# NikolaZubic/2dimageto3dmodel

Hardware: NVIDIA H100
Metric: render+loss+GAN images/sec (cfg3: cfg2 render+loss at batch 32 + conv-GAN 256x256 G/D iteration, 1 G : 2 D, Adam) (higher is better)
Workload: dtype tf32 (convs) / f32

## Files before the change

2dimageto3dmodel_b200/csrc/b3d_core.cu:

```cuda
#include <atomic>
#include <stdarg.h>
#include <string.h>

#include "b3d_common.cuh"

namespace b3d {
static thread_local char g_err[512] = "";
static thread_local char g_variant[256] = "";
static std::atomic<uint64_t> g_launches{0};

void set_error(const char* fmt, ...) {
    va_list ap;
    va_start(ap, fmt);
    vsnprintf(g_err, sizeof(g_err), fmt, ap);
    va_end(ap);
}
void clear_variant() { g_variant[0] = 0; }
void add_variant(const char* fmt, ...) {
    size_t n = strlen(g_variant);
    if (n + 2 >= sizeof(g_variant)) return;
    if (n) g_variant[n++] = ';';
    va_list ap;
    va_start(ap, fmt);
    vsnprintf(g_variant + n, sizeof(g_variant) - n, fmt, ap);
    va_end(ap);
}
void count_launch(int n) { g_launches.fetch_add((uint64_t)n, std::memory_order_relaxed); }
}

extern "C" {
const char* b3d_last_error(void) { return b3d::g_err; }
const char* b3d_last_variant(void) { return b3d::g_variant; }
int b3d_version(void) { return 420; }
uint64_t b3d_launch_count(void) { return b3d::g_launches.load(std::memory_order_relaxed); }
}
```

2dimageto3dmodel_b200/csrc/tc_common.cuh:

```cuda
#pragma once
#include <cuda.h>
#include <cuda_runtime.h>
#include <stdint.h>

#include "b3d_common.cuh"

namespace tc {

__device__ __forceinline__ uint32_t smem_u32(const void* p) { return (uint32_t)__cvta_generic_to_shared(p); }

__device__ __forceinline__ void mbar_init(uint64_t* bar, uint32_t count) {
    asm volatile("mbarrier.init.shared::cta.b64 [%0], %1;" ::"r"(smem_u32(bar)), "r"(count));
}
__device__ __forceinline__ void fence_barrier_init() { asm volatile("fence.mbarrier_init.release.cluster;" ::: "memory"); }
__device__ __forceinline__ void fence_proxy_async() { asm volatile("fence.proxy.async.shared::cta;" ::: "memory"); }

__device__ __forceinline__ void mbar_arrive_expect_tx(uint64_t* bar, uint32_t bytes) {
    asm volatile("mbarrier.arrive.expect_tx.shared::cta.b64 _, [%0], %1;" ::"r"(smem_u32(bar)), "r"(bytes) : "memory");
}
__device__ __forceinline__ void mbar_arrive(uint64_t* bar) {
    asm volatile("mbarrier.arrive.shared::cta.b64 _, [%0];" ::"r"(smem_u32(bar)) : "memory");
}
__device__ __forceinline__ void mbar_arrive(uint64_t* bar, uint32_t count) {
    asm volatile("mbarrier.arrive.shared::cta.b64 _, [%0], %1;" ::"r"(smem_u32(bar)), "r"(count) : "memory");
// ... 52 lines not shown
    return v;
}
__device__ __forceinline__ float lds_f32(uint32_t smem_addr) {
    float v;
    asm volatile("ld.shared.f32 %0, [%1];" : "=f"(v) : "r"(smem_addr) : "memory");
    return v;
}
__device__ __forceinline__ float2 lds_f32x2(uint32_t smem_addr) {
    float2 v;
    asm volatile("ld.shared.v2.f32 {%0, %1}, [%2];" : "=f"(v.x), "=f"(v.y) : "r"(smem_addr) : "memory");
    return v;
}
__device__ __forceinline__ float4 lds_f32x4(uint32_t smem_addr) {
    float4 v;
    asm volatile("ld.shared.v4.f32 {%0, %1, %2, %3}, [%4];" : "=f"(v.x), "=f"(v.y), "=f"(v.z), "=f"(v.w) : "r"(smem_addr) : "memory");
    return v;
}
__device__ __forceinline__ void sts_f32x4(uint32_t smem_addr, float a, float b, float c, float d) {
    asm volatile("st.shared.v4.f32 [%0], {%1, %2, %3, %4};" ::"r"(smem_addr), "f"(a), "f"(b), "f"(c), "f"(d) : "memory");
}
__device__ __forceinline__ void fence_operand(uint32_t& r) { asm volatile("" : "+r"(r)::"memory"); }
__device__ __forceinline__ void fence_operand(float& r) { asm volatile("" : "+f"(r)::"memory"); }
template <int N>
__device__ __forceinline__ void setmaxnreg_dec() { asm volatile("setmaxnreg.dec.sync.aligned.u32 %0;" ::"n"(N)); }
template <int N>
__device__ __forceinline__ void setmaxnreg_inc() { asm volatile("setmaxnreg.inc.sync.aligned.u32 %0;" ::"n"(N)); }

template <int N>
struct Wgmma;
template <>
struct Wgmma<64> {
    __device__ __forceinline__ static void mma_rs(float (&d)[32], const uint32_t (&a)[4], uint64_t db, uint32_t accumulate) {
        asm volatile(
            "{\n"
            ".reg .pred p;\n"
            "setp.ne.b32 p, %37, 0;\n"
            "wgmma.mma_async.sync.aligned.m64n64k8.f32.tf32.tf32 "
            "{%0, %1, %2, %3, %4, %5, %6, %7, %8, %9, %10, %11, %12, %13, %14, %15, %16, %17, %18, %19, %20, %21, %22, %23, %24, %25, %26, %27, %28, %29, %30, %31}, "
            "{%32, %33, %34, %35}, %36, p, 1, 1;\n"
            "}\n"
            : "+f"(d[0]), "+f"(d[1]), "+f"(d[2]), "+f"(d[3]), "+f"(d[4]), "+f"(d[5]), "+f"(d[6]), "+f"(d[7]), "+f"(d[8]), "+f"(d[9]), "+f"(d[10]), "+f"(d[11]), "+f"(d[12]), "+f"(d[13]), "+f"(d[14]), "+f"(d[15]), "+f"(d[16]), "+f"(d[17]), "+f"(d[18]), "+f"(d[19]), "+f"(d[20]), "+f"(d[21]), "+f"(d[22]), "+f"(d[23]), "+f"(d[24]), "+f"(d[25]), "+f"(d[26]), "+f"(d[27]), "+f"(d[28]), "+f"(d[29]), "+f"(d[30]), "+f"(d[31])
            : "r"(a[0]), "r"(a[1]), "r"(a[2]), "r"(a[3]), "l"(db), "r"(accumulate));
    }
    __device__ __forceinline__ static void mma(float (&d)[32], uint64_t da, uint64_t db, uint32_t accumulate) {
        asm volatile(
            "{\n"
            ".reg .pred p;\n"
            "setp.ne.b32 p, %34, 0;\n"
            "wgmma.mma_async.sync.aligned.m64n64k8.f32.tf32.tf32 "
            "{%0, %1, %2, %3, %4, %5, %6, %7, %8, %9, %10, %11, %12, %13, %14, %15, %16, %17, %18, %19, %20, %21, %22, %23, %24, %25, %26, %27, %28, %29, %30, %31}, "
            "%32, %33, p, 1, 1;\n"
            "}\n"
            : "+f"(d[0]), "+f"(d[1]), "+f"(d[2]), "+f"(d[3]), "+f"(d[4]), "+f"(d[5]), "+f"(d[6]), "+f"(d[7]), "+f"(d[8]), "+f"(d[9]), "+f"(d[10]), "+f"(d[11]), "+f"(d[12]), "+f"(d[13]), "+f"(d[14]), "+f"(d[15]), "+f"(d[16]), "+f"(d[17]), "+f"(d[18]), "+f"(d[19]), "+f"(d[20]), "+f"(d[21]), "+f"(d[22]), "+f"(d[23]), "+f"(d[24]), "+f"(d[25]), "+f"(d[26]), "+f"(d[27]), "+f"(d[28]), "+f"(d[29]), "+f"(d[30]), "+f"(d[31])
            : "l"(da), "l"(db), "r"(accumulate));
    }
};
template <>
struct Wgmma<128> {
    __device__ __forceinline__ static void mma_rs(float (&d)[64], const uint32_t (&a)[4], uint64_t db, uint32_t accumulate) {
        asm volatile(
            "{\n"
            ".reg .pred p;\n"
            "setp.ne.b32 p, %69, 0;\n"
            "wgmma.mma_async.sync.aligned.m64n128k8.f32.tf32.tf32 "
            "{%0, %1, %2, %3, %4, %5, %6, %7, %8, %9, %10, %11, %12, %13, %14, %15, %16, %17, %18, %19, %20, %21, %22, %23, %24, %25, %26, %27, %28, %29, %30, %31, %32, %33, %34, %35, %36, %37, %38, %39, %40, %41, %42, %43, %44, %45, %46, %47, %48, %49, %50, %51, %52, %53, %54, %55, %56, %57, %58, %59, %60, %61, %62, %63}, "
            "{%64, %65, %66, %67}, %68, p, 1, 1;\n"
            "}\n"
            : "+f"(d[0]), "+f"(d[1]), "+f"(d[2]), "+f"(d[3]), "+f"(d[4]), "+f"(d[5]), "+f"(d[6]), "+f"(d[7]), "+f"(d[8]), "+f"(d[9]), "+f"(d[10]), "+f"(d[11]), "+f"(d[12]), "+f"(d[13]), "+f"(d[14]), "+f"(d[15]), "+f"(d[16]), "+f"(d[17]), "+f"(d[18]), "+f"(d[19]), "+f"(d[20]), "+f"(d[21]), "+f"(d[22]), "+f"(d[23]), "+f"(d[24]), "+f"(d[25]), "+f"(d[26]), "+f"(d[27]), "+f"(d[28]), "+f"(d[29]), "+f"(d[30]), "+f"(d[31]), "+f"(d[32]), "+f"(d[33]), "+f"(d[34]), "+f"(d[35]), "+f"(d[36]), "+f"(d[37]), "+f"(d[38]), "+f"(d[39]), "+f"(d[40]), "+f"(d[41]), "+f"(d[42]), "+f"(d[43]), "+f"(d[44]), "+f"(d[45]), "+f"(d[46]), "+f"(d[47]), "+f"(d[48]), "+f"(d[49]), "+f"(d[50]), "+f"(d[51]), "+f"(d[52]), "+f"(d[53]), "+f"(d[54]), "+f"(d[55]), "+f"(d[56]), "+f"(d[57]), "+f"(d[58]), "+f"(d[59]), "+f"(d[60]), "+f"(d[61]), "+f"(d[62]), "+f"(d[63])
            : "r"(a[0]), "r"(a[1]), "r"(a[2]), "r"(a[3]), "l"(db), "r"(accumulate));
    }
    __device__ __forceinline__ static void mma(float (&d)[64], uint64_t da, uint64_t db, uint32_t accumulate) {
        asm volatile(
            "{\n"
            ".reg .pred p;\n"
            "setp.ne.b32 p, %66, 0;\n"
            "wgmma.mma_async.sync.aligned.m64n128k8.f32.tf32.tf32 "
            "{%0, %1, %2, %3, %4, %5, %6, %7, %8, %9, %10, %11, %12, %13, %14, %15, %16, %17, %18, %19, %20, %21, %22, %23, %24, %25, %26, %27, %28, %29, %30, %31, %32, %33, %34, %35, %36, %37, %38, %39, %40, %41, %42, %43, %44, %45, %46, %47, %48, %49, %50, %51, %52, %53, %54, %55, %56, %57, %58, %59, %60, %61, %62, %63}, "
            "%64, %65, p, 1, 1;\n"
            "}\n"
            : "+f"(d[0]), "+f"(d[1]), "+f"(d[2]), "+f"(d[3]), "+f"(d[4]), "+f"(d[5]), "+f"(d[6]), "+f"(d[7]), "+f"(d[8]), "+f"(d[9]), "+f"(d[10]), "+f"(d[11]), "+f"(d[12]), "+f"(d[13]), "+f"(d[14]), "+f"(d[15]), "+f"(d[16]), "+f"(d[17]), "+f"(d[18]), "+f"(d[19]), "+f"(d[20]), "+f"(d[21]), "+f"(d[22]), "+f"(d[23]), "+f"(d[24]), "+f"(d[25]), "+f"(d[26]), "+f"(d[27]), "+f"(d[28]), "+f"(d[29]), "+f"(d[30]), "+f"(d[31]), "+f"(d[32]), "+f"(d[33]), "+f"(d[34]), "+f"(d[35]), "+f"(d[36]), "+f"(d[37]), "+f"(d[38]), "+f"(d[39]), "+f"(d[40]), "+f"(d[41]), "+f"(d[42]), "+f"(d[43]), "+f"(d[44]), "+f"(d[45]), "+f"(d[46]), "+f"(d[47]), "+f"(d[48]), "+f"(d[49]), "+f"(d[50]), "+f"(d[51]), "+f"(d[52]), "+f"(d[53]), "+f"(d[54]), "+f"(d[55]), "+f"(d[56]), "+f"(d[57]), "+f"(d[58]), "+f"(d[59]), "+f"(d[60]), "+f"(d[61]), "+f"(d[62]), "+f"(d[63])
            : "l"(da), "l"(db), "r"(accumulate));
    }
};
__device__ __forceinline__ uint64_t desc_k128(uint32_t smem_addr) {
    uint64_t d = 0;
    d |= (uint64_t)((smem_addr & 0x3FFFF) >> 4);
    d |= (uint64_t)1 << 16;
    d |= (uint64_t)(1024 >> 4) << 32;
    d |= (uint64_t)1 << 62;
    return d;
}
__device__ __forceinline__ uint64_t desc_k32(uint32_t smem_addr) {
    uint64_t d = 0;
    d |= (uint64_t)((smem_addr & 0x3FFFF) >> 4);
    d |= (uint64_t)1 << 16;
    d |= (uint64_t)(256 >> 4) << 32;
    d |= (uint64_t)3 << 62;
    return d;
}

typedef CUresult (*EncodeTiledFn)(CUtensorMap*, CUtensorMapDataType, cuuint32_t, void*, const cuuint64_t*,
                                  const cuuint64_t*, const cuuint32_t*, const cuuint32_t*, CUtensorMapInterleave,
                                  CUtensorMapSwizzle, CUtensorMapL2promotion, CUtensorMapFloatOOBfill);

inline EncodeTiledFn encode_fn() {
    static EncodeTiledFn fn = nullptr;
    if (!fn) {
        void* p = nullptr;
        cudaDriverEntryPointQueryResult q;
        if (cudaGetDriverEntryPoint("cuTensorMapEncodeTiled", &p, cudaEnableDefault, &q) == cudaSuccess &&
            q == cudaDriverEntryPointSuccess)
            fn = reinterpret_cast<EncodeTiledFn>(p);
    }
    return fn;
}

inline int make_tmap_f32(CUtensorMap* m, const void* base, int rank, const uint64_t* dims, const uint64_t* strides_b,
                         const uint32_t* box, const uint32_t* elem_strides = nullptr,
                         CUtensorMapSwizzle swz = CU_TENSOR_MAP_SWIZZLE_128B) {
    EncodeTiledFn fn = encode_fn();
    if (!fn) {
        b3d::set_error("cuTensorMapEncodeTiled is not available from the driver");
        return B3D_ECUDA;
    }
    cuuint64_t gd[5], gs[5];
    cuuint32_t bx[5], es[5];
    for (int i = 0; i < rank; ++i) {
        gd[i] = dims[i];
        bx[i] = box[i];
        es[i] = elem_strides ? elem_strides[i] : 1;
        if (i > 0) gs[i - 1] = strides_b[i - 1];
    }
    CUresult r = fn(m, CU_TENSOR_MAP_DATA_TYPE_FLOAT32, (cuuint32_t)rank, const_cast<void*>(base), gd, gs, bx, es,
                    CU_TENSOR_MAP_INTERLEAVE_NONE, swz, CU_TENSOR_MAP_L2_PROMOTION_L2_256B,
                    CU_TENSOR_MAP_FLOAT_OOB_FILL_NONE);
    if (r != CUDA_SUCCESS) {
        b3d::set_error("cuTensorMapEncodeTiled failed with CUresult %d (rank %d, inner box %u)", (int)r, rank, box[0]);
        return B3D_ECUDA;
    }
    return B3D_OK;
}

inline int num_sms() {
    int dev = 0, n = 0;
    if (cudaGetDevice(&dev) != cudaSuccess || cudaDeviceGetAttribute(&n, cudaDevAttrMultiProcessorCount, dev) != cudaSuccess || n < 1)
        return 132;
    return n;
}

}
```

2dimageto3dmodel_b200/csrc/tc_conv.cu:

```cuda
#include "tc_common.cuh"

namespace {

constexpr int BM = 128;
constexpr int BK = 32;
constexpr int MMA_K = 8;
constexpr int MAX_TAPS = 25;
constexpr int NTHREADS = 384;

struct ConvParams {
    int N, Hout, Wout, Cout;
    int BW, BH, BI;
    int tiles_x, tiles_y;
    int xbase;
    int ntaps, kslices;
    int sy, sx;
    int dy[MAX_TAPS], dx[MAX_TAPS];
    int wtap[MAX_TAPS];
    int OH, OW, OC, osy, osx;
    float leaky;
    double* stats;
    int fold;
    int fold_y0;
    int mask;
// ... 420 lines not shown
    const int wg = threadIdx.x >> 7, tid = threadIdx.x & 127;

    if (wg == 0) {
        tc::setmaxnreg_dec<80>();
        auto issue = [&](int j) {
            if (tid != 0) return;
            const long long k = k_lo + j;
            const int n = (int)(k / per_img), rem = (int)(k % per_img);
            const int x0 = (rem % p.kx) * p.BWk, y0 = (rem / p.kx) * p.BHk;
            const int rb = j % NRAW;
            unsigned char* dst = raw + rb * S::RAW_BYTES;
            tc::mbar_wait(rawempty + rb, ((j / NRAW) & 1) ^ 1);
            tc::mbar_arrive_expect_tx(rawfull + rb, S::DY_BYTES + S::RAW_X);
            tc::tma_load_5d(dst, &tmap_dy, rawfull + rb, 0, x0, y0, n, co0 / 32);
            tc::tma_load_5d(dst + S::DY_BYTES, &tmap_x, rawfull + rb, 0, p.st * x0 + s + p.xoff, p.st * y0 + r - p.pad_y, n, ci0 / 32);
        };
        for (int j = 0; j < NRAW - 1 && j < KI; ++j) issue(j);
        const uint32_t raw_s = tc::smem_u32(raw), base_s = tc::smem_u32(base);
        for (int it = 0; it < KI; ++it) {
            if (it + NRAW - 1 < KI) issue(it + NRAW - 1);
            const int rb = it % NRAW, st = it % STAGES;
            tc::mbar_wait(rawfull + rb, (it / NRAW) & 1);
            tc::mbar_wait(empty + st, ((it / STAGES) & 1) ^ 1);
            wgrad_transpose<BN, T, S::WROWS>(raw_s + rb * S::RAW_BYTES + S::DY_BYTES, base_s + st * S::STAGE_BYTES, tid);
            tc::fence_proxy_async();
            tc::mbar_arrive(full + st);
            tc::named_sync(2, 128);
        }
        return;
    }
    tc::setmaxnreg_inc<208>();

    const int h = wg - 1, lane = tid & 31;
    if (h >= nact) return;
    int aoff[4];
#pragma unroll
    for (int e = 0; e < 4; ++e)
        aoff[e] = dy_tile_offset(h * 64 + wgrad_row_co((tid >> 5) * 16 + (lane >> 2) + 8 * (e & 1)), (lane & 3) + 4 * (e >> 1));
    float acc[T][BN / 2];
#pragma unroll
    for (int t = 0; t < T; ++t)
#pragma unroll
        for (int i = 0; i < BN / 2; ++i) acc[t][i] = 0.f;
    wgrad_consume<BN, T, STAGES, NRAW, S::RAW_BYTES, S::STAGE_BYTES>(acc, tc::smem_u32(raw), tc::smem_u32(base), full, empty, rawfull,
                                                                     rawempty, aoff, 0, 1, KI, tid, true);
    if (KI == 0) return;
    const int m_a = (tid >> 5) * 16 + (lane >> 2);
    const int cq = ci0 + 2 * (lane & 3);
#pragma unroll
    for (int t = 0; t < T; ++t) {
        const int sc = s + t * p.tstep;
#pragma unroll
        for (int e = 0; e < 2; ++e) {
            const int co = co0 + h * 64 + wgrad_row_co(m_a + 8 * e);
            if (co >= p.Cout) continue;
#pragma unroll
            for (int j = 0; j < BN / 8; ++j) {
                const int ci = cq + 8 * j;
                if (ci >= p.Cin) continue;
                const float v0 = acc[t][4 * j + 2 * e], v1 = acc[t][4 * j + 2 * e + 1];
                if (p.tapmajor) {
                    atomicAdd(reinterpret_cast<float2*>(dw + ((size_t)(r * p.kw + sc) * p.Cout + co) * p.Cin + ci), make_float2(v0, v1));
                } else {
                    atomicAdd(dw + (((size_t)co * p.Cin + ci) * p.kh + r) * p.kw + sc, v0);
                    atomicAdd(dw + (((size_t)co * p.Cin + ci + 1) * p.kh + r) * p.kw + sc, v1);
                }
            }
        }
    }
}

template <int BN, int STAGES, int NRAW, int T>
int launch_wgrad(const CUtensorMap& mdy, const CUtensorMap& mx, const WgradParams& p, float* dw, dim3 grid, cudaStream_t st) {
    using S = WSmem<BN, STAGES, NRAW, T>;
    static_assert(S::TOTAL <= 227 * 1024, "wgrad pipeline does not fit shared memory");
    B3D_CUDA_OK(cudaFuncSetAttribute(wgrad_wgmma_kernel<BN, STAGES, NRAW, T>, cudaFuncAttributeMaxDynamicSharedMemorySize, S::TOTAL));
    wgrad_wgmma_kernel<BN, STAGES, NRAW, T><<<grid, NTHREADS, S::TOTAL, st>>>(mdy, mx, p, dw);
    B3D_LAUNCH_OK();
    b3d::add_variant("wgrad_wgmma<%d,%d,%d,%d>", BN, STAGES, NRAW, T);
    return B3D_OK;
}

constexpr int STEM_KW = 5, STEM_STAGES = 4, STEM_NRAW = 3;
constexpr int STEM_BATCH = 3;
struct StemSmem {
    static constexpr int DY_BYTES = 64 * BK * 4;
    static constexpr int WPX = BK + STEM_KW - 1;
    static constexpr int RAW_X_MAX = 8 * WPX * 32;
    static constexpr int RAW_BYTES = (DY_BYTES + RAW_X_MAX + 1023) / 1024 * 1024;
    static constexpr int TILE_BYTES = 64 * BK * 4;
    static constexpr int STAGE_BYTES = STEM_KW * TILE_BYTES;
    static constexpr int TOTAL = STEM_STAGES * STAGE_BYTES + STEM_NRAW * RAW_BYTES + 1024 + 256;
};

__global__ void __launch_bounds__(NTHREADS, 1)
wgrad_stem_kernel(const __grid_constant__ CUtensorMap tmap_dy, const __grid_constant__ CUtensorMap tmap_x,
                  const WgradParams p, int fold_kh, float* __restrict__ dw) {
    using S = StemSmem;
    extern __shared__ unsigned char smem_raw[];
    unsigned char* base = reinterpret_cast<unsigned char*>((reinterpret_cast<uintptr_t>(smem_raw) + 1023) & ~uintptr_t(1023));
    unsigned char* raw = base + STEM_STAGES * S::STAGE_BYTES;
    uint64_t* full = reinterpret_cast<uint64_t*>(raw + STEM_NRAW * S::RAW_BYTES);
    uint64_t* empty = full + STEM_STAGES;
    uint64_t* rawfull = empty + STEM_STAGES;
    uint64_t* rawempty = rawfull + STEM_NRAW;

    const int co0 = blockIdx.x * 64, split = blockIdx.y;
    const int per_img = p.kx * p.ky;
    const long long ktotal = (long long)p.N * per_img;
    const long long k_lo = ktotal * split / p.splits, k_hi = ktotal * (split + 1) / p.splits;
    const int KI = (int)(k_hi - k_lo);
    const int creal = 8 * fold_kh;
    const int xbytes = fold_kh * S::WPX * 32;

    if (threadIdx.x == 0) {
        tc::tma_prefetch_desc(&tmap_dy);
        tc::tma_prefetch_desc(&tmap_x);
        for (int i = 0; i < STEM_STAGES; ++i) {
            tc::mbar_init(full + i, 128);
            tc::mbar_init(empty + i, 1);
        }
        for (int i = 0; i < STEM_NRAW; ++i) {
            tc::mbar_init(rawfull + i, 1);
            tc::mbar_init(rawempty + i, 4);
        }
        tc::fence_barrier_init();
    }
    __syncthreads();
    const int wg = threadIdx.x >> 7, tid = threadIdx.x & 127;

    if (wg == 0) {
        tc::setmaxnreg_dec<56>();
        auto issue = [&](int j) {
            if (tid != 0) return;
            const long long k = k_lo + j;
            const int n = (int)(k / per_img), rem = (int)(k % per_img);
            const int x0 = (rem % p.kx) * BK, y0 = rem / p.kx;
            const int rb = j % STEM_NRAW;
            unsigned char* dst = raw + rb * S::RAW_BYTES;
            tc::mbar_wait(rawempty + rb, ((j / STEM_NRAW) & 1) ^ 1);
            tc::mbar_arrive_expect_tx(rawfull + rb, S::DY_BYTES + xbytes);
            tc::tma_load_5d(dst, &tmap_dy, rawfull + rb, 0, x0, y0, n, co0 / 32);
            tc::tma_load_4d(dst + S::DY_BYTES, &tmap_x, rawfull + rb, 0, x0, y0 - p.pad_y, n);
        };
        for (int i = tid; i < STEM_STAGES * STEM_KW * (64 - creal) * 8; i += 128) {
            const int c = creal + (i >> 3) % (64 - creal), tile = (i >> 3) / (64 - creal);
            *reinterpret_cast<float4*>(base + tile * S::TILE_BYTES + c * 128 + (i & 7) * 16) = make_float4(0.f, 0.f, 0.f, 0.f);
        }
        for (int j = 0; j < STEM_NRAW - 1 && j < KI; ++j) issue(j);
        const int ntask = fold_kh * 8 * STEM_KW * 8;
        const uint32_t raw_s = tc::smem_u32(raw), base_s = tc::smem_u32(base);
        for (int it = 0; it < KI; ++it) {
            if (it + STEM_NRAW - 1 < KI) issue(it + STEM_NRAW - 1);
            const int rb = it % STEM_NRAW, st = it % STEM_STAGES;
            tc::mbar_wait(rawfull + rb, (it / STEM_NRAW) & 1);
            tc::mbar_wait(empty + st, ((it / STEM_STAGES) & 1) ^ 1);
            const uint32_t src = raw_s + rb * S::RAW_BYTES + S::DY_BYTES;
            const uint32_t dst = base_s + st * S::STAGE_BYTES;
            for (int i0 = tid; i0 < ntask; i0 += STEM_BATCH * 128) {
                float v[STEM_BATCH][4];
                uint32_t d[STEM_BATCH];
#pragma unroll
                for (int g = 0; g < STEM_BATCH; ++g) {
                    const int i = i0 + 128 * g;
                    if (i >= ntask) break;
                    const int ci = i & 7, u = i >> 3;
                    const int s = u % STEM_KW, q = (u / STEM_KW) & 7, r = u / (STEM_KW * 8);
                    const uint32_t a = src + ((r * S::WPX + 4 * q + s) * 8 + ci) * 4;
#pragma unroll
                    for (int e = 0; e < 4; ++e) v[g][e] = tc::lds_f32(a + 32 * e);
                    d[g] = dst + s * S::TILE_BYTES + (8 * r + ci) * 128 + ((q ^ ci) << 4);
                }
#pragma unroll
                for (int g = 0; g < STEM_BATCH; ++g) {
                    if (i0 + 128 * g >= ntask) break;
                    tc::sts_f32x4(d[g], v[g][0], v[g][1], v[g][2], v[g][3]);
                }
            }
            tc::fence_proxy_async();
            tc::mbar_arrive(full + st);
            tc::named_sync(2, 128);
        }
        return;
    }
    tc::setmaxnreg_inc<224>();

    const int h = wg - 1, lane = tid & 31;
    int aoff[4];
#pragma unroll
    for (int e = 0; e < 4; ++e)
        aoff[e] = dy_tile_offset(wgrad_row_co((tid >> 5) * 16 + (lane >> 2) + 8 * (e & 1)), (lane & 3) + 4 * (e >> 1));
    float acc[STEM_KW][32];
#pragma unroll
    for (int t = 0; t < STEM_KW; ++t)
#pragma unroll
        for (int i = 0; i < 32; ++i) acc[t][i] = 0.f;
    static_assert(S::TILE_BYTES == 64 * 128, "a tap's B tile is 64 channel rows of 128 bytes");
    wgrad_consume<64, STEM_KW, STEM_STAGES, STEM_NRAW, S::RAW_BYTES, S::STAGE_BYTES>(acc, tc::smem_u32(raw), tc::smem_u32(base), full, empty,
                                                                                     rawfull, rawempty, aoff, h, 2, KI, tid, false);
    if (h >= KI) return;
    const int m_a = (tid >> 5) * 16 + (lane >> 2);
#pragma unroll
    for (int t = 0; t < STEM_KW; ++t) {
#pragma unroll
        for (int e = 0; e < 2; ++e) {
            const int co = co0 + wgrad_row_co(m_a + 8 * e);
#pragma unroll
            for (int j = 0; j < 8; ++j) {
                const int ci = 8 * j + 2 * (lane & 3);
                if (ci >= creal) continue;
                const float v0 = acc[t][4 * j + 2 * e], v1 = acc[t][4 * j + 2 * e + 1];
                if (p.tapmajor) {
                    atomicAdd(reinterpret_cast<float2*>(dw + ((size_t)t * p.Cout + co) * p.Cin + ci), make_float2(v0, v1));
                } else {
                    atomicAdd(dw + ((size_t)co * p.Cin + ci) * STEM_KW + t, v0);
                    atomicAdd(dw + ((size_t)co * p.Cin + ci + 1) * STEM_KW + t, v1);
                }
            }
        }
    }
}

int wgrad_splits(int base_ctas, long long ktotal) {
    constexpr long long FIXED = 16;
    const long long sms = tc::num_sms();
    long long smax = ktotal / 8;
    if (smax > 8 * sms) smax = 8 * sms;
    int best = 1;
    long long best_cost = -1;
    for (long long s = 1; s <= smax; ++s) {
        const long long cost = (base_ctas * s + sms - 1) / sms * ((ktotal + s - 1) / s + FIXED);
        if (best_cost < 0 || cost < best_cost) { best = (int)s; best_cost = cost; }
    }
    return best;
}

template <int BN, int STAGES, int KW = 1>
int launch_conv(const CUtensorMap& mx, const CUtensorMap& mw, const CUtensorMap& mm, const ConvParams& p, const float* bias, float* out,
                int tiles, cudaStream_t st) {
    using S = CSmem<BN, STAGES, KW>;
    static_assert(S::TOTAL <= 227 * 1024, "conv pipeline does not fit shared memory");
    B3D_CUDA_OK(cudaFuncSetAttribute(conv_wgmma_kernel<BN, STAGES, KW>, cudaFuncAttributeMaxDynamicSharedMemorySize, S::TOTAL));
    const int work = tiles * b3d::ceil_div(p.Cout, BN) * p.ncls;
    const int sms = tc::num_sms();
    conv_wgmma_kernel<BN, STAGES, KW><<<work < sms ? work : sms, NTHREADS, S::TOTAL, st>>>(mx, mw, mm, p, bias, out, tiles, work);
    B3D_LAUNCH_OK();
    if (KW > 1) b3d::add_variant("conv_wgmma_rowwin<%d,%d,%d>", BN, KW, STAGES);
    else b3d::add_variant("conv_wgmma<%d,%d>", BN, STAGES);
    return B3D_OK;
}

template <int BN>
int launch_rowwin(int kw, const CUtensorMap& mx, const CUtensorMap& mw, const CUtensorMap& mm, const ConvParams& p, const float* bias,
                  float* out, int tiles, cudaStream_t st) {
    if (kw == 2) return launch_conv<BN, BN == 64 ? 5 : 4, 2>(mx, mw, mm, p, bias, out, tiles, st);
    if (kw == 3) return launch_conv<BN, BN == 64 ? 4 : 3, 3>(mx, mw, mm, p, bias, out, tiles, st);
    return launch_conv<BN, BN == 64 ? 3 : 2, 5>(mx, mw, mm, p, bias, out, tiles, st);
}

int pow2_floor(int v) {
    int p = 1;
    while (p * 2 <= v) p *= 2;
    return p;
}

}

extern "C" {

int b3d_conv2d_tf32(const float* x, const float* wt, const float* bias, float* out, int N, int H, int W, int Cin,
                    int Hout, int Wout, int Cout, int ntaps, const int* dy, const int* dx, int sy, int sx, int OH,
                    int OW, int OC, int osy, int osx, int ooy, int oox, float leaky, const int* wtap,
                    int wtaps_total, double* stats, int fold_kh, int fold_pad, const b3d_conv_opts* opts, void* stream) {
    B3D_REQUIRE(N > 0 && H > 0 && W > 0 && Hout > 0 && Wout > 0 && Cout > 0, B3D_EINVAL, "b3d_conv2d_tf32: bad sizes");
    B3D_REQUIRE(Cin > 0 && Cin % BK == 0, B3D_EINVAL, "b3d_conv2d_tf32: Cin=%d must be a multiple of %d", Cin, BK);
    B3D_REQUIRE(ntaps >= 1 && ntaps <= MAX_TAPS && dy && dx, B3D_EINVAL, "b3d_conv2d_tf32: bad taps");
    B3D_REQUIRE(x && wt && out, B3D_EINVAL, "b3d_conv2d_tf32: null pointer");
    B3D_REQUIRE(sy >= 1 && sy <= 2 && sx >= 1 && sx <= 2, B3D_EINVAL, "b3d_conv2d_tf32: stride must be 1 or 2");
    if (!wtap) wtaps_total = ntaps;
    B3D_REQUIRE(wtaps_total >= ntaps || wtap, B3D_EINVAL, "b3d_conv2d_tf32: bad weight tap count");
    for (int t = 0; wtap && t < ntaps; ++t)
        B3D_REQUIRE(wtap[t] >= 0 && wtap[t] < wtaps_total, B3D_EINVAL, "b3d_conv2d_tf32: weight tap %d out of range", wtap[t]);
    B3D_CHECK_ALIGNED(x);
    B3D_CHECK_ALIGNED(wt);
    b3d::clear_variant();

    const float* mask = opts ? opts->mask : nullptr;
    const float mslope = opts ? opts->mask_slope : 1.f;
    B3D_REQUIRE(!mask || (reinterpret_cast<uintptr_t>(mask) % 16 == 0 && OC % 4 == 0), B3D_EINVAL,
                "b3d_conv2d_tf32: the mask needs a 16-byte aligned base and OC %% 4 == 0 (OC=%d)", OC);
    const int stats_sum = (opts && opts->stats_sum_only) ? 1 : 0;
    const int xpitch = (opts && opts->x_row_pitch) ? opts->x_row_pitch : W;
    const int ncls = (opts && opts->nclass > 1) ? opts->nclass : 1;
    B3D_REQUIRE(ncls <= 4 && ntaps % ncls == 0 && (ncls == 1 || (sy == 1 && sx == 1 && fold_kh == 0)), B3D_EINVAL,
                "b3d_conv2d_tf32: nclass=%d needs <= 4 equal tap groups of a stride-1 launch", ncls);
    const int tpc = ntaps / ncls;
    int cooy[4] = {ooy, ooy, ooy, ooy}, coox[4] = {oox, oox, oox, oox};
    for (int c = 0; c < ncls && ncls > 1; ++c) { cooy[c] = opts->class_ooy[c]; coox[c] = opts->class_oox[c]; }
    B3D_REQUIRE(xpitch >= W && (fold_kh == 0 || xpitch == W), B3D_EINVAL, "b3d_conv2d_tf32: x_row_pitch=%d must be >= W=%d (and absent with the on-the-fly fold)", xpitch, W);
    if (fold_kh > 0) {
        B3D_REQUIRE(fold_kh <= 8 && Cin == 32 * ((8 * fold_kh + 31) / 32) && sy == 1 && sx == 1 && !wtap && Wout % BM == 0,
                    B3D_EINVAL, "b3d_conv2d_tf32: on-the-fly fold needs 8 input channels, stride 1 and Wout %% 128 == 0 (Wout=%d)", Wout);
    }
// ... 59 lines not shown
            if (int rc = tc::make_tmap_f32(&mm, mask, 4, dims, strides, box, es)) return rc;
        }
        CUtensorMap mx;
        if (g_kw && wspan >= BM) {
            p.dx0 = g_step > 0 ? dx[0] : dx[g_kw - 1];
            for (int t = 0; t < g_kw; ++t) p.shift[t] = dx[t] - p.dx0;
            const uint64_t dims[4] = {(uint64_t)Cin, (uint64_t)W, (uint64_t)H, (uint64_t)N};
            const uint64_t strides[3] = {(uint64_t)Cin * 4, (uint64_t)xpitch * Cin * 4, (uint64_t)H * xpitch * Cin * 4};
            const uint32_t box[4] = {(uint32_t)BK, (uint32_t)(BM + g_kw - 1), 1, 1};
            if (int rc = tc::make_tmap_f32(&mx, x, 4, dims, strides, box)) return rc;
            CUtensorMap mwr;
            const uint64_t wdims[3] = {(uint64_t)Cin, (uint64_t)Cout, (uint64_t)wtaps_total};
            const uint64_t wstrides[2] = {(uint64_t)Cin * 4, (uint64_t)Cout * Cin * 4};
            const uint32_t wbox[3] = {(uint32_t)BK, (uint32_t)BN, (uint32_t)((g_kw - 1) * g_wstep + 1)};
            const uint32_t wes[3] = {1, 1, (uint32_t)g_wstep};
            if (int rc = tc::make_tmap_f32(&mwr, wt, 3, wdims, wstrides, wbox, wes)) return rc;
            return BN == 128 ? launch_rowwin<128>(g_kw, mx, mwr, mm, p, bias, out, tiles, st)
                             : launch_rowwin<64>(g_kw, mx, mwr, mm, p, bias, out, tiles, st);
        }
        if (fold_kh > 0) {
            B3D_REQUIRE(p.BH == 1 && p.BI == 1, B3D_EINVAL, "b3d_conv2d_tf32: on-the-fly fold needs one-row tiles");
            const uint64_t dims[4] = {8, (uint64_t)W, (uint64_t)H, (uint64_t)N};
            const uint64_t strides[3] = {32, (uint64_t)W * 32, (uint64_t)H * W * 32};
            const uint32_t box[4] = {8, (uint32_t)p.BW, 4, 1};
            if (int rc = tc::make_tmap_f32(&mx, x, 4, dims, strides, box, nullptr, CU_TENSOR_MAP_SWIZZLE_32B)) return rc;
        } else {
            const uint64_t dims[4] = {(uint64_t)Cin, (uint64_t)W, (uint64_t)H, (uint64_t)N};
            const uint64_t strides[3] = {(uint64_t)Cin * 4, (uint64_t)xpitch * Cin * 4, (uint64_t)H * xpitch * Cin * 4};
            const uint32_t box[4] = {(uint32_t)BK, (uint32_t)(sx * (p.BW - 1) + 1), (uint32_t)(sy * (p.BH - 1) + 1), (uint32_t)p.BI};
            const uint32_t es[4] = {1, (uint32_t)sx, (uint32_t)sy, 1};
            if (int rc = tc::make_tmap_f32(&mx, x, 4, dims, strides, box, es)) return rc;
        }
        if (BN == 256) return launch_conv<256, 4>(mx, mw, mm, p, bias, out, tiles, st);
        if (BN == 128) return launch_conv<128, 6>(mx, mw, mm, p, bias, out, tiles, st);
        return launch_conv<64, 8>(mx, mw, mm, p, bias, out, tiles, st);
    };
    const int bw_full = pow2_floor(Wout < BM ? Wout : BM);
    const int rem = Wout % bw_full;
    if (rem != 0 && rem * 8 <= bw_full && Wout > bw_full) {
        const int rc = run(0, Wout - rem);
        return rc ? rc : run(Wout - rem, Wout);
    }
    return run(0, Wout);
}

int b3d_conv2d_wgrad_tf32(const float* dy, const float* x, float* dw, int N, int H, int W, int Cin, int Hout, int Wout,
                          int Cout, int kh, int kw, int pad_y, int stride, int x_off, int tap_major, int fold_kh, int dy_row_pitch,
                          void* stream) {
    B3D_REQUIRE(N > 0 && Cin > 0 && Cout > 0 && H > 0 && W > 0 && Hout > 0 && Wout > 0, B3D_EINVAL,
                "b3d_conv2d_wgrad_tf32: bad sizes");
    B3D_REQUIRE(kh * kw <= MAX_TAPS && (stride == 1 || stride == 2) && x_off >= 0, B3D_EINVAL, "b3d_conv2d_wgrad_tf32: bad kernel/stride");
    B3D_REQUIRE(dy && x && dw, B3D_EINVAL, "b3d_conv2d_wgrad_tf32: null pointer");
    B3D_REQUIRE(Cin % 32 == 0 && Cout % 32 == 0, B3D_EINVAL,
                "b3d_conv2d_wgrad_tf32: Cin=%d and Cout=%d must be multiples of 32 (pad the channels with zeros)", Cin, Cout);
    B3D_CHECK_ALIGNED(dy);
    B3D_CHECK_ALIGNED(x);
    b3d::clear_variant();
    if (tap_major) B3D_CHECK_ALIGNED(dw);
    WgradParams p{};
    p.N = N; p.Hout = Hout; p.Wout = Wout; p.Cout = Cout; p.Cin = Cin;
    const uint64_t dpitch = dy_row_pitch > 0 ? dy_row_pitch : Wout;
    B3D_REQUIRE(dpitch >= (uint64_t)Wout, B3D_EINVAL, "b3d_conv2d_wgrad_tf32: dy_row_pitch=%d must be >= Wout=%d", dy_row_pitch, Wout);
    cudaStream_t st = (cudaStream_t)stream;
    if (fold_kh > 0) {
        B3D_REQUIRE(fold_kh > 4 && fold_kh <= 8 && Cin == 64 && kh == 1 && kw == STEM_KW && stride == 1 && x_off == 0 &&
                        Cout % 64 == 0 && W == Wout + STEM_KW - 1 && Hout == H + 2 * pad_y - fold_kh + 1,
                    B3D_EINVAL, "b3d_conv2d_wgrad_tf32: the raw-input stem weight gradient needs 4 < fold_kh <= 8 rows folded into "
                    "64 channels, a 1x5 stride-1 filter, Cout %% 64 == 0 and the x padding in the input");
        p.BWk = BK; p.BHk = 1;
        p.kx = b3d::ceil_div(Wout, BK);
        p.ky = Hout;
        p.kh = 1; p.kw = kw; p.pad_y = pad_y; p.st = 1; p.tapmajor = tap_major ? 1 : 0;
        p.splits = wgrad_splits(Cout / 64, (long long)N * p.kx * p.ky);
        CUtensorMap mdy, mx;
        {
            const uint64_t dims[5] = {32, (uint64_t)Wout, (uint64_t)Hout, (uint64_t)N, (uint64_t)Cout / 32};
            const uint64_t strides[4] = {(uint64_t)Cout * 4, dpitch * Cout * 4, (uint64_t)Hout * dpitch * Cout * 4, 128};
            const uint32_t box[5] = {32, (uint32_t)BK, 1, 1, 2};
            if (int rc = tc::make_tmap_f32(&mdy, dy, 5, dims, strides, box)) return rc;
        }
        {
            const uint64_t dims[4] = {8, (uint64_t)W, (uint64_t)H, (uint64_t)N};
            const uint64_t strides[3] = {32, (uint64_t)W * 32, (uint64_t)H * W * 32};
            const uint32_t box[4] = {8, (uint32_t)StemSmem::WPX, (uint32_t)fold_kh, 1};
            if (int rc = tc::make_tmap_f32(&mx, x, 4, dims, strides, box, nullptr, CU_TENSOR_MAP_SWIZZLE_NONE)) return rc;
        }
        B3D_CUDA_OK(cudaFuncSetAttribute(wgrad_stem_kernel, cudaFuncAttributeMaxDynamicSharedMemorySize, StemSmem::TOTAL));
        wgrad_stem_kernel<<<dim3(Cout / 64, p.splits), NTHREADS, StemSmem::TOTAL, st>>>(mdy, mx, p, fold_kh, dw);
        B3D_LAUNCH_OK();
        b3d::add_variant("wgrad_stem<%d,%d,%d>", STEM_KW, STEM_STAGES, STEM_NRAW);
        return B3D_OK;
    }
    p.BWk = pow2_floor(Wout < BK ? Wout : BK);
    p.BHk = BK / p.BWk;
    p.kx = b3d::ceil_div(Wout, p.BWk);
    p.ky = b3d::ceil_div(Hout, p.BHk);
    p.kh = kh; p.kw = kw; p.pad_y = pad_y; p.st = stride; p.xoff = x_off; p.tapmajor = tap_major ? 1 : 0;
    const int BN = Cin > 64 ? 128 : 64;
    int T = 1;
    p.tstep = 1;
    if (Wout >= BK) {
        if (stride == 1 && kw == 3 && BN == 64) T = 3;
        if (stride == 2 && kw == 4) { T = 2; p.tstep = 2; }
    }
    const int base_ctas = b3d::ceil_div(Cout, BM) * b3d::ceil_div(Cin, BN) * kh * (kw / T);
    const long long ktotal = (long long)N * p.kx * p.ky;
    const int splits = wgrad_splits(base_ctas, ktotal);
    p.splits = splits;

    CUtensorMap mdy, mx;
    {
        const uint64_t dims[5] = {32, (uint64_t)Wout, (uint64_t)Hout, (uint64_t)N, (uint64_t)Cout / 32};
        const uint64_t strides[4] = {(uint64_t)Cout * 4, dpitch * Cout * 4, (uint64_t)Hout * dpitch * Cout * 4, 128};
        const uint32_t box[5] = {32, (uint32_t)p.BWk, (uint32_t)p.BHk, 1, (uint32_t)(BM / 32)};
        if (int rc = tc::make_tmap_f32(&mdy, dy, 5, dims, strides, box)) return rc;
    }
    {
        const uint64_t dims[5] = {32, (uint64_t)W, (uint64_t)H, (uint64_t)N, (uint64_t)Cin / 32};
        const uint64_t strides[4] = {(uint64_t)Cin * 4, (uint64_t)W * Cin * 4, (uint64_t)H * W * Cin * 4, 128};
        const int wpx = T == 1 ? p.BWk : 36;
        const uint32_t box[5] = {32, (uint32_t)(stride * (wpx - 1) + 1), (uint32_t)(stride * (p.BHk - 1) + 1), 1, (uint32_t)(BN / 32)};
        const uint32_t es[5] = {1, (uint32_t)stride, (uint32_t)stride, 1, 1};
        if (int rc = tc::make_tmap_f32(&mx, x, 5, dims, strides, box, es, CU_TENSOR_MAP_SWIZZLE_NONE)) return rc;
    }
    dim3 grid(b3d::ceil_div(Cout, BM), b3d::ceil_div(Cin, BN), kh * (kw / T) * splits);
    if (T == 3) return launch_wgrad<64, 3, 3, 3>(mdy, mx, p, dw, grid, st);
    if (T == 2) return BN == 128 ? launch_wgrad<128, 2, 3, 2>(mdy, mx, p, dw, grid, st) : launch_wgrad<64, 3, 3, 2>(mdy, mx, p, dw, grid, st);
    if (BN == 128) return launch_wgrad<128, 3, 3, 1>(mdy, mx, p, dw, grid, st);
    return launch_wgrad<64, 4, 4, 1>(mdy, mx, p, dw, grid, st);
}

}
```

Baseline: 1451.

## Size stem wgrad WGMMA N to the real folded channel count

```diff
diff --git a/2dimageto3dmodel_b200/csrc/b3d_core.cu b/2dimageto3dmodel_b200/csrc/b3d_core.cu
--- a/2dimageto3dmodel_b200/csrc/b3d_core.cu
+++ b/2dimageto3dmodel_b200/csrc/b3d_core.cu
@@ -31,6 +31,6 @@
 extern "C" {
 const char* b3d_last_error(void) { return b3d::g_err; }
 const char* b3d_last_variant(void) { return b3d::g_variant; }
-int b3d_version(void) { return 420; }
+int b3d_version(void) { return 430; }
 uint64_t b3d_launch_count(void) { return b3d::g_launches.load(std::memory_order_relaxed); }
 }
diff --git a/2dimageto3dmodel_b200/csrc/tc_common.cuh b/2dimageto3dmodel_b200/csrc/tc_common.cuh
--- a/2dimageto3dmodel_b200/csrc/tc_common.cuh
+++ b/2dimageto3dmodel_b200/csrc/tc_common.cuh
@@ -158,6 +158,51 @@
             : "l"(da), "l"(db), "r"(accumulate));
     }
 };
+template <>
+struct Wgmma<40> {
+    __device__ __forceinline__ static void mma_rs(float (&d)[20], const uint32_t (&a)[4], uint64_t db, uint32_t accumulate) {
+        asm volatile(
+            "{\n"
+            ".reg .pred p;\n"
+            "setp.ne.b32 p, %25, 0;\n"
+            "wgmma.mma_async.sync.aligned.m64n40k8.f32.tf32.tf32 "
+            "{%0, %1, %2, %3, %4, %5, %6, %7, %8, %9, %10, %11, %12, %13, %14, %15, %16, %17, %18, %19}, "
+            "{%20, %21, %22, %23}, %24, p, 1, 1;\n"
+            "}\n"
+            : "+f"(d[0]), "+f"(d[1]), "+f"(d[2]), "+f"(d[3]), "+f"(d[4]), "+f"(d[5]), "+f"(d[6]), "+f"(d[7]), "+f"(d[8]), "+f"(d[9]), "+f"(d[10]), "+f"(d[11]), "+f"(d[12]), "+f"(d[13]), "+f"(d[14]), "+f"(d[15]), "+f"(d[16]), "+f"(d[17]), "+f"(d[18]), "+f"(d[19])
+            : "r"(a[0]), "r"(a[1]), "r"(a[2]), "r"(a[3]), "l"(db), "r"(accumulate));
+    }
+};
+template <>
+struct Wgmma<48> {
+    __device__ __forceinline__ static void mma_rs(float (&d)[24], const uint32_t (&a)[4], uint64_t db, uint32_t accumulate) {
+        asm volatile(
+            "{\n"
+            ".reg .pred p;\n"
+            "setp.ne.b32 p, %29, 0;\n"
+            "wgmma.mma_async.sync.aligned.m64n48k8.f32.tf32.tf32 "
+            "{%0, %1, %2, %3, %4, %5, %6, %7, %8, %9, %10, %11, %12, %13, %14, %15, %16, %17, %18, %19, %20, %21, %22, %23}, "
+            "{%24, %25, %26, %27}, %28, p, 1, 1;\n"
+            "}\n"
+            : "+f"(d[0]), "+f"(d[1]), "+f"(d[2]), "+f"(d[3]), "+f"(d[4]), "+f"(d[5]), "+f"(d[6]), "+f"(d[7]), "+f"(d[8]), "+f"(d[9]), "+f"(d[10]), "+f"(d[11]), "+f"(d[12]), "+f"(d[13]), "+f"(d[14]), "+f"(d[15]), "+f"(d[16]), "+f"(d[17]), "+f"(d[18]), "+f"(d[19]), "+f"(d[20]), "+f"(d[21]), "+f"(d[22]), "+f"(d[23])
+            : "r"(a[0]), "r"(a[1]), "r"(a[2]), "r"(a[3]), "l"(db), "r"(accumulate));
+    }
+};
+template <>
+struct Wgmma<56> {
+    __device__ __forceinline__ static void mma_rs(float (&d)[28], const uint32_t (&a)[4], uint64_t db, uint32_t accumulate) {
+        asm volatile(
+            "{\n"
+            ".reg .pred p;\n"
+            "setp.ne.b32 p, %33, 0;\n"
+            "wgmma.mma_async.sync.aligned.m64n56k8.f32.tf32.tf32 "
+            "{%0, %1, %2, %3, %4, %5, %6, %7, %8, %9, %10, %11, %12, %13, %14, %15, %16, %17, %18, %19, %20, %21, %22, %23, %24, %25, %26, %27}, "
+            "{%28, %29, %30, %31}, %32, p, 1, 1;\n"
+            "}\n"
+            : "+f"(d[0]), "+f"(d[1]), "+f"(d[2]), "+f"(d[3]), "+f"(d[4]), "+f"(d[5]), "+f"(d[6]), "+f"(d[7]), "+f"(d[8]), "+f"(d[9]), "+f"(d[10]), "+f"(d[11]), "+f"(d[12]), "+f"(d[13]), "+f"(d[14]), "+f"(d[15]), "+f"(d[16]), "+f"(d[17]), "+f"(d[18]), "+f"(d[19]), "+f"(d[20]), "+f"(d[21]), "+f"(d[22]), "+f"(d[23]), "+f"(d[24]), "+f"(d[25]), "+f"(d[26]), "+f"(d[27])
+            : "r"(a[0]), "r"(a[1]), "r"(a[2]), "r"(a[3]), "l"(db), "r"(accumulate));
+    }
+};
 __device__ __forceinline__ uint64_t desc_k128(uint32_t smem_addr) {
     uint64_t d = 0;
     d |= (uint64_t)((smem_addr & 0x3FFFF) >> 4);
diff --git a/2dimageto3dmodel_b200/csrc/tc_conv.cu b/2dimageto3dmodel_b200/csrc/tc_conv.cu
--- a/2dimageto3dmodel_b200/csrc/tc_conv.cu
+++ b/2dimageto3dmodel_b200/csrc/tc_conv.cu
@@ -526,21 +526,23 @@
 }
 
 constexpr int STEM_KW = 5, STEM_STAGES = 4, STEM_NRAW = 3;
-constexpr int STEM_BATCH = 3;
+constexpr int STEM_WPX = BK + STEM_KW - 1;
+template <int N>
 struct StemSmem {
     static constexpr int DY_BYTES = 64 * BK * 4;
-    static constexpr int WPX = BK + STEM_KW - 1;
-    static constexpr int RAW_X_MAX = 8 * WPX * 32;
-    static constexpr int RAW_BYTES = (DY_BYTES + RAW_X_MAX + 1023) / 1024 * 1024;
-    static constexpr int TILE_BYTES = 64 * BK * 4;
+    static constexpr int RAW_X = N * STEM_WPX * 4;
+    static constexpr int RAW_BYTES = (DY_BYTES + RAW_X + 1023) / 1024 * 1024;
+    static constexpr int TILE_BYTES = N * BK * 4;
     static constexpr int STAGE_BYTES = STEM_KW * TILE_BYTES;
     static constexpr int TOTAL = STEM_STAGES * STAGE_BYTES + STEM_NRAW * RAW_BYTES + 1024 + 256;
+    static_assert(TILE_BYTES % 1024 == 0, "B tiles start on a swizzle-atom boundary");
 };
 
+template <int N>
 __global__ void __launch_bounds__(NTHREADS, 1)
 wgrad_stem_kernel(const __grid_constant__ CUtensorMap tmap_dy, const __grid_constant__ CUtensorMap tmap_x,
-                  const WgradParams p, int fold_kh, float* __restrict__ dw) {
-    using S = StemSmem;
+                  const WgradParams p, float* __restrict__ dw) {
+    using S = StemSmem<N>;
     extern __shared__ unsigned char smem_raw[];
     unsigned char* base = reinterpret_cast<unsigned char*>((reinterpret_cast<uintptr_t>(smem_raw) + 1023) & ~uintptr_t(1023));
     unsigned char* raw = base + STEM_STAGES * S::STAGE_BYTES;
@@ -554,8 +556,6 @@
     const long long ktotal = (long long)p.N * per_img;
     const long long k_lo = ktotal * split / p.splits, k_hi = ktotal * (split + 1) / p.splits;
     const int KI = (int)(k_hi - k_lo);
-    const int creal = 8 * fold_kh;
-    const int xbytes = fold_kh * S::WPX * 32;
 
     if (threadIdx.x == 0) {
         tc::tma_prefetch_desc(&tmap_dy);
@@ -583,42 +583,34 @@
             const int rb = j % STEM_NRAW;
             unsigned char* dst = raw + rb * S::RAW_BYTES;
             tc::mbar_wait(rawempty + rb, ((j / STEM_NRAW) & 1) ^ 1);
-            tc::mbar_arrive_expect_tx(rawfull + rb, S::DY_BYTES + xbytes);
+            tc::mbar_arrive_expect_tx(rawfull + rb, S::DY_BYTES + S::RAW_X);
             tc::tma_load_5d(dst, &tmap_dy, rawfull + rb, 0, x0, y0, n, co0 / 32);
             tc::tma_load_4d(dst + S::DY_BYTES, &tmap_x, rawfull + rb, 0, x0, y0 - p.pad_y, n);
         };
-        for (int i = tid; i < STEM_STAGES * STEM_KW * (64 - creal) * 8; i += 128) {
-            const int c = creal + (i >> 3) % (64 - creal), tile = (i >> 3) / (64 - creal);
-            *reinterpret_cast<float4*>(base + tile * S::TILE_BYTES + c * 128 + (i & 7) * 16) = make_float4(0.f, 0.f, 0.f, 0.f);
-        }
         for (int j = 0; j < STEM_NRAW - 1 && j < KI; ++j) issue(j);
-        const int ntask = fold_kh * 8 * STEM_KW * 8;
+        const int c = tid & 1, q = (tid >> 1) & 7, r = tid >> 4;
+        const uint32_t src_t = ((r * STEM_WPX + 4 * q) * 8 + 4 * c) * 4;
+        const uint32_t dst_t = (8 * r + 4 * c) * 128;
         const uint32_t raw_s = tc::smem_u32(raw), base_s = tc::smem_u32(base);
         for (int it = 0; it < KI; ++it) {
             if (it + STEM_NRAW - 1 < KI) issue(it + STEM_NRAW - 1);
             const int rb = it % STEM_NRAW, st = it % STEM_STAGES;
             tc::mbar_wait(rawfull + rb, (it / STEM_NRAW) & 1);
             tc::mbar_wait(empty + st, ((it / STEM_STAGES) & 1) ^ 1);
-            const uint32_t src = raw_s + rb * S::RAW_BYTES + S::DY_BYTES;
-            const uint32_t dst = base_s + st * S::STAGE_BYTES;
-            for (int i0 = tid; i0 < ntask; i0 += STEM_BATCH * 128) {
-                float v[STEM_BATCH][4];
-                uint32_t d[STEM_BATCH];
-#pragma unroll
-                for (int g = 0; g < STEM_BATCH; ++g) {
-                    const int i = i0 + 128 * g;
-                    if (i >= ntask) break;
-                    const int ci = i & 7, u = i >> 3;
-                    const int s = u % STEM_KW, q = (u / STEM_KW) & 7, r = u / (STEM_KW * 8);
-                    const uint32_t a = src + ((r * S::WPX + 4 * q + s) * 8 + ci) * 4;
-#pragma unroll
-                    for (int e = 0; e < 4; ++e) v[g][e] = tc::lds_f32(a + 32 * e);
-                    d[g] = dst + s * S::TILE_BYTES + (8 * r + ci) * 128 + ((q ^ ci) << 4);
-                }
-#pragma unroll
-                for (int g = 0; g < STEM_BATCH; ++g) {
-                    if (i0 + 128 * g >= ntask) break;
-                    tc::sts_f32x4(d[g], v[g][0], v[g][1], v[g][2], v[g][3]);
+            if (tid < 2 * N) {
+                const uint32_t src = raw_s + rb * S::RAW_BYTES + S::DY_BYTES + src_t;
+                const uint32_t dst = base_s + st * S::STAGE_BYTES + dst_t;
+#pragma unroll
+                for (int hc = 0; hc < 2; ++hc) {
+                    float2 v[8];
+#pragma unroll
+                    for (int u = 0; u < 8; ++u) v[u] = tc::lds_f32x2(src + 32 * u + 8 * hc);
+#pragma unroll
+                    for (int s = 0; s < STEM_KW; ++s) {
+                        const uint32_t d = dst + s * S::TILE_BYTES + 2 * hc * 128;
+                        tc::sts_f32x4(d + ((q ^ (4 * c + 2 * hc)) << 4), v[s].x, v[s + 1].x, v[s + 2].x, v[s + 3].x);
+                        tc::sts_f32x4(d + 128 + ((q ^ (4 * c + 2 * hc + 1)) << 4), v[s].y, v[s + 1].y, v[s + 2].y, v[s + 3].y);
+                    }
                 }
             }
             tc::fence_proxy_async();
@@ -634,13 +626,13 @@
 #pragma unroll
     for (int e = 0; e < 4; ++e)
         aoff[e] = dy_tile_offset(wgrad_row_co((tid >> 5) * 16 + (lane >> 2) + 8 * (e & 1)), (lane & 3) + 4 * (e >> 1));
-    float acc[STEM_KW][32];
+    float acc[STEM_KW][N / 2];
 #pragma unroll
     for (int t = 0; t < STEM_KW; ++t)
 #pragma unroll
-        for (int i = 0; i < 32; ++i) acc[t][i] = 0.f;
-    static_assert(S::TILE_BYTES == 64 * 128, "a tap's B tile is 64 channel rows of 128 bytes");
-    wgrad_consume<64, STEM_KW, STEM_STAGES, STEM_NRAW, S::RAW_BYTES, S::STAGE_BYTES>(acc, tc::smem_u32(raw), tc::smem_u32(base), full, empty,
+        for (int i = 0; i < N / 2; ++i) acc[t][i] = 0.f;
+    static_assert(S::TILE_BYTES == N * 128, "a tap's B tile is N channel rows of 128 bytes");
+    wgrad_consume<N, STEM_KW, STEM_STAGES, STEM_NRAW, S::RAW_BYTES, S::STAGE_BYTES>(acc, tc::smem_u32(raw), tc::smem_u32(base), full, empty,
                                                                                      rawfull, rawempty, aoff, h, 2, KI, tid, false);
     if (h >= KI) return;
     const int m_a = (tid >> 5) * 16 + (lane >> 2);
@@ -650,9 +642,8 @@
         for (int e = 0; e < 2; ++e) {
             const int co = co0 + wgrad_row_co(m_a + 8 * e);
 #pragma unroll
-            for (int j = 0; j < 8; ++j) {
+            for (int j = 0; j < N / 8; ++j) {
                 const int ci = 8 * j + 2 * (lane & 3);
-                if (ci >= creal) continue;
                 const float v0 = acc[t][4 * j + 2 * e], v1 = acc[t][4 * j + 2 * e + 1];
                 if (p.tapmajor) {
                     atomicAdd(reinterpret_cast<float2*>(dw + ((size_t)t * p.Cout + co) * p.Cin + ci), make_float2(v0, v1));
@@ -663,6 +654,17 @@
             }
         }
     }
+}
+
+template <int N>
+int launch_wgrad_stem(const CUtensorMap& mdy, const CUtensorMap& mx, const WgradParams& p, float* dw, dim3 grid, cudaStream_t st) {
+    using S = StemSmem<N>;
+    static_assert(S::TOTAL <= 227 * 1024, "stem wgrad pipeline does not fit shared memory");
+    B3D_CUDA_OK(cudaFuncSetAttribute(wgrad_stem_kernel<N>, cudaFuncAttributeMaxDynamicSharedMemorySize, S::TOTAL));
+    wgrad_stem_kernel<N><<<grid, NTHREADS, S::TOTAL, st>>>(mdy, mx, p, dw);
+    B3D_LAUNCH_OK();
+    b3d::add_variant("wgrad_stem<%d,%d,%d>", STEM_KW, STEM_STAGES, STEM_NRAW);
+    return B3D_OK;
 }
 
 int wgrad_splits(int base_ctas, long long ktotal) {
@@ -888,14 +890,14 @@
         {
             const uint64_t dims[4] = {8, (uint64_t)W, (uint64_t)H, (uint64_t)N};
             const uint64_t strides[3] = {32, (uint64_t)W * 32, (uint64_t)H * W * 32};
-            const uint32_t box[4] = {8, (uint32_t)StemSmem::WPX, (uint32_t)fold_kh, 1};
+            const uint32_t box[4] = {8, (uint32_t)STEM_WPX, (uint32_t)fold_kh, 1};
             if (int rc = tc::make_tmap_f32(&mx, x, 4, dims, strides, box, nullptr, CU_TENSOR_MAP_SWIZZLE_NONE)) return rc;
         }
-        B3D_CUDA_OK(cudaFuncSetAttribute(wgrad_stem_kernel, cudaFuncAttributeMaxDynamicSharedMemorySize, StemSmem::TOTAL));
-        wgrad_stem_kernel<<<dim3(Cout / 64, p.splits), NTHREADS, StemSmem::TOTAL, st>>>(mdy, mx, p, fold_kh, dw);
-        B3D_LAUNCH_OK();
-        b3d::add_variant("wgrad_stem<%d,%d,%d>", STEM_KW, STEM_STAGES, STEM_NRAW);
-        return B3D_OK;
+        const dim3 grid(Cout / 64, p.splits);
+        if (fold_kh == 5) return launch_wgrad_stem<40>(mdy, mx, p, dw, grid, st);
+        if (fold_kh == 6) return launch_wgrad_stem<48>(mdy, mx, p, dw, grid, st);
+        if (fold_kh == 7) return launch_wgrad_stem<56>(mdy, mx, p, dw, grid, st);
+        return launch_wgrad_stem<64>(mdy, mx, p, dw, grid, st);
     }
     p.BWk = pow2_floor(Wout < BK ? Wout : BK);
     p.BHk = BK / p.BWk;
```

Measured after the change: 1464 (median of 6 runs). About the same (+0.9%).
